# facebookresearch/videoseal

Hardware: AMD Instinct MI355X
Metric: frames/sec embed+extract 256-bit @768x768 (higher is better)
Workload: dtype f32 (2 x f16 operand split, 3 products on v_mfma_f32_32x32x16_f16, fp32 accumulate); 1 GPU; videoseal_1.0 256-bit, 32 frames 768x768 per GPU, image mode (embedder on every frame, full-res JND), embed + detect; card=videoseal_1.0, weights=random-init (seeded), no checkpoint offline, batch_per_gpu=32, mode=image

## Files before the change

### videoseal_amd/csrc/net_ops.hip

```cpp
#include <algorithm>
#include <cstdlib>
#include <cstring>

#include "conv_common.h"

namespace {

__global__ __launch_bounds__(256) void layernorm_act_kernel(const float* __restrict__ x, int64_t rows, int C, int64_t ld,
                                                            const float* __restrict__ w, const float* __restrict__ b,
                                                            float eps, int act, float* __restrict__ out, int64_t out_ld) {
  const int lane = threadIdx.x & 63;
  const int64_t row = (int64_t)blockIdx.x * 4 + (threadIdx.x >> 6);
  if (row >= rows) return;
  const float* xr = x + row * ld;
  float s = 0.f;
  for (int c = lane; c < C; c += 64) s += xr[c];
  const float mean = wave_sum(s) / (float)C;
  float v = 0.f;
  for (int c = lane; c < C; c += 64) {
    const float dlt = xr[c] - mean;
    v += dlt * dlt;
  }
  const float var = wave_sum(v) / (float)C;
  const float den = sqrtf(var + eps);
  float* orow = out + row * out_ld;
  for (int c = lane; c < (int)out_ld; c += 64) {
    float y = 0.f;
    if (c < C) y = vs_apply_act(w[c] * ((xr[c] - mean) / den) + b[c], act);
    orow[c] = y;
  }
}

template <int LPP, int VMAX>
__global__ __launch_bounds__(256) void layernorm_act_lanes_kernel(const float* __restrict__ x, int64_t rows, int C, int64_t ld,
                                                                  const float* __restrict__ w, const float* __restrict__ b, float eps, int act,
                                                                  float* __restrict__ out, int64_t out_ld, int pH, int pW) {
  constexpr int RPB = 256 / LPP;
  const int q = threadIdx.x & (LPP - 1);
  const int64_t row = (int64_t)blockIdx.x * RPB + (threadIdx.x / LPP);
  bool live = row < rows;
  const int C4 = (C + 3) >> 2, O4 = (int)(out_ld >> 2);
  const float* xr = x + (live ? row : rows - 1) * ld;
  f32x4 v[VMAX];
  float s = 0.f;
#pragma unroll
  for (int k = 0; k < VMAX; ++k) {
    const int c4 = q + k * LPP;
    v[k] = f32x4{0.f, 0.f, 0.f, 0.f};
    if (c4 < C4) {
      v[k] = *reinterpret_cast<const f32x4*>(xr + 4 * c4);
#pragma unroll
      for (int e = 0; e < 4; ++e)
        if (4 * c4 + e < C) s += v[k][e];
    }
  }
#pragma unroll
  for (int o = LPP / 2; o > 0; o >>= 1) s += __shfl_xor(s, o, 64);
  const float mean = s / (float)C;
  float qv = 0.f;
#pragma unroll
  for (int k = 0; k < VMAX; ++k) {
    const int c4 = q + k * LPP;
    if (c4 < C4) {
#pragma unroll
      for (int e = 0; e < 4; ++e)
        if (4 * c4 + e < C) { const float dlt = v[k][e] - mean; qv += dlt * dlt; }
    }
  }
#pragma unroll
  for (int o = LPP / 2; o > 0; o >>= 1) qv += __shfl_xor(qv, o, 64);
  const float den = sqrtf(qv / (float)C + eps);
  float* orow = out + row * out_ld;
  if (pW > 0 && live) {
    const int px = (int)(row % pW);
    const int64_t t = row / pW;
    const int py = (int)(t % pH);
    const int64_t fb = t / pH;
    const int oh = pH >> 1, ow = pW >> 1;
    live = (py >> 1) < oh && (px >> 1) < ow;
    orow = out + ((fb * oh + (py >> 1)) * ow + (px >> 1)) * (4 * (int64_t)C) + ((py & 1) * 2 + (px & 1)) * C;
  }
  if (!live) return;
#pragma unroll
  for (int k = 0; k < VMAX; ++k) {
    const int c4 = q + k * LPP;
    if (c4 < O4) {
      f32x4 o = {0.f, 0.f, 0.f, 0.f};
// ... 505 lines not shown

template <int CG>
__global__ __launch_bounds__(256) void upconv_gather_ln_kernel(const float* __restrict__ z, int64_t zld, int H, int W, int Co,
                                                               int tpp_log2, const float* __restrict__ lnw,
                                                               const float* __restrict__ lnb, float eps, int act,
                                                               float* __restrict__ out, int64_t old, int64_t npix, int nblk) {
  const int per = (nblk + 7) >> 3;
  const int64_t vb = (int64_t)(blockIdx.x & 7) * per + (blockIdx.x >> 3);
  const int64_t gid = vb * 256 + threadIdx.x;
  const int64_t pq = gid >> tpp_log2;
  const int g = (int)(gid & ((1 << tpp_log2) - 1));
  const bool live = pq < npix && vb < nblk;
  const int64_t p = live ? pq : 0;
  constexpr int NVP = CG / 4;
  f32x4 lwv[NVP], lbv[NVP];
#pragma unroll
  for (int j = 0; j < NVP; ++j) {
    lwv[j] = *reinterpret_cast<const f32x4*>(lnw + g * CG + 4 * j);
    lbv[j] = *reinterpret_cast<const f32x4*>(lnb + g * CG + 4 * j);
  }
  const int W2 = 2 * W, H2 = 2 * H;
  const int X = (int)(p % W2);
  const int64_t t0 = p / W2;
  const int Y = (int)(t0 % H2);
  const int64_t b = t0 / H2;
  int ys[3][2], xs[3][2];
  float wy[3][2], wx[3][2];
#pragma unroll
  for (int k = 0; k < 3; ++k) {
    int yr = Y + k - 1, xr = X + k - 1;
    yr = yr < 0 ? -yr : (yr >= H2 ? 2 * H2 - 2 - yr : yr);
    xr = xr < 0 ? -xr : (xr >= W2 ? 2 * W2 - 2 - xr : xr);
    const float sy = fmaxf((yr + 0.5f) * 0.5f - 0.5f, 0.f), sx = fmaxf((xr + 0.5f) * 0.5f - 0.5f, 0.f);
    const int y0 = (int)sy, x0 = (int)sx;
    ys[k][0] = y0; ys[k][1] = y0 + (y0 < H - 1);
    xs[k][0] = x0; xs[k][1] = x0 + (x0 < W - 1);
    wy[k][1] = sy - y0; wy[k][0] = 1.f - wy[k][1];
    wx[k][1] = sx - x0; wx[k][0] = 1.f - wx[k][1];
  }
  constexpr int NV = CG / 4;
  f32x4 acc[NV];
#pragma unroll
  for (int j = 0; j < NV; ++j) acc[j] = f32x4{0.f, 0.f, 0.f, 0.f};
  const float* zb = z + b * H * W * zld + g * CG;
#pragma unroll
  for (int ky = 0; ky < 3; ++ky)
#pragma unroll
    for (int a = 0; a < 2; ++a) {
      const float* zr = zb + (int64_t)ys[ky][a] * W * zld + ky * 3 * Co;
#pragma unroll
      for (int kx = 0; kx < 3; ++kx)
#pragma unroll
        for (int c = 0; c < 2; ++c) {
          const float w = wy[ky][a] * wx[kx][c];
          const float* q = zr + (int64_t)xs[kx][c] * zld + kx * Co;
#pragma unroll
          for (int j = 0; j < NV; ++j) acc[j] += w * *reinterpret_cast<const f32x4*>(q + 4 * j);
        }
    }
  float s = 0.f;
#pragma unroll
  for (int j = 0; j < NV; ++j) s += (acc[j][0] + acc[j][1]) + (acc[j][2] + acc[j][3]);
  for (int o = 1; o < (1 << tpp_log2); o <<= 1) s += __shfl_xor(s, o, 64);
  const float mean = s / (float)Co;
  float v = 0.f;
#pragma unroll
  for (int j = 0; j < NV; ++j)
#pragma unroll
    for (int e = 0; e < 4; ++e) { const float dl = acc[j][e] - mean; v += dl * dl; }
  for (int o = 1; o < (1 << tpp_log2); o <<= 1) v += __shfl_xor(v, o, 64);
  const float den = sqrtf(v / (float)Co + eps);
  if (!live) return;
  float* orow = out + p * old + g * CG;
#pragma unroll
  for (int j = 0; j < NV; ++j) {
    const f32x4 wv = lwv[j], bv = lbv[j];
    f32x4 o;
#pragma unroll
    for (int e = 0; e < 4; ++e) o[e] = vs_apply_act(wv[e] * ((acc[j][e] - mean) / den) + bv[e], act);
    *reinterpret_cast<f32x4*>(orow + 4 * j) = o;
  }
}

__global__ __launch_bounds__(256) void im2col3x3_kernel(const float* __restrict__ x, int H, int W, int64_t ld, int reflect,
                                                        float* __restrict__ out, int64_t total) {
  const int G = (int)(ld >> 2);
  for (int64_t i = (int64_t)blockIdx.x * 256 + threadIdx.x; i < total; i += (int64_t)gridDim.x * 256) {
    const int cg = (int)(i % G);
    int64_t r = i / G;
    const int t = (int)(r % 9);
    r /= 9;
    const int xx = (int)(r % W);
    const int yy = (int)((r / W) % H);
    const int64_t b = r / ((int64_t)W * H);
    int sy = yy + t / 3 - 1, sx = xx + t % 3 - 1;
    bool ok = true;
    if (reflect) {
      sy = sy < 0 ? -sy : (sy >= H ? 2 * H - 2 - sy : sy);
      sx = sx < 0 ? -sx : (sx >= W ? 2 * W - 2 - sx : sx);
    } else {
      ok = sy >= 0 && sy < H && sx >= 0 && sx < W;
    }
    f32x4 v = {0.f, 0.f, 0.f, 0.f};
    if (ok) v = *reinterpret_cast<const f32x4*>(x + ((b * H + sy) * W + sx) * ld + cg * 4);
    *reinterpret_cast<f32x4*>(out + (r * 9 + t) * ld + cg * 4) = v;
  }
}

__global__ __launch_bounds__(256) void msg_pre_kernel(const float* __restrict__ P, int N, float* __restrict__ T, int64_t total) {
  for (int64_t i = (int64_t)blockIdx.x * 256 + threadIdx.x; i < total; i += (int64_t)gridDim.x * 256) {
    const int n = (int)(i % N);
    const int cls = (int)((i / N) % 9);
    const int64_t bm = i / ((int64_t)9 * N);
    const int cy = cls / 3, cx = cls % 3;
    const float* pb = P + bm * 9 * N + n;
    float v = 0.f;
    for (int ky = (cy == 0 ? 1 : 0); ky <= (cy == 2 ? 1 : 2); ++ky)
      for (int kx = (cx == 0 ? 1 : 0); kx <= (cx == 2 ? 1 : 2); ++kx) v += pb[(ky * 3 + kx) * N];
    T[i] = v;
  }
}

__global__ __launch_bounds__(256) void cat2_scale_kernel(const float* __restrict__ x, int C1, int64_t ld1, const float* __restrict__ skip,
                                                         int C2, int64_t ld2, float s, int64_t rows, float* __restrict__ out,
                                                         int64_t old) {
  const int g1 = x ? C1 >> 2 : 0, G = g1 + (C2 >> 2);
  const int64_t total = rows * G;
  for (int64_t i = (int64_t)blockIdx.x * 256 + threadIdx.x; i < total; i += (int64_t)gridDim.x * 256) {
    const int cg = (int)(i % G);
    const int64_t r = i / G;
    f32x4 v;
    int c;
    if (cg < g1) { c = cg * 4; v = *reinterpret_cast<const f32x4*>(x + r * ld1 + c); }
    else { const int c2 = (cg - g1) * 4; c = C1 + c2; v = *reinterpret_cast<const f32x4*>(skip + r * ld2 + c2) * s; }
    *reinterpret_cast<f32x4*>(out + r * old + c) = v;
  }
}

__global__ __launch_bounds__(256) void msg_latent_kernel(const float* __restrict__ table, const int32_t* __restrict__ msgs,
                                                         int nbits, int hidden, float* __restrict__ lat) {
  __shared__ int rowsel[1024];
  const int b = blockIdx.y;
  for (int k = threadIdx.x; k < nbits; k += 256) rowsel[k] = 2 * k + (msgs[(int64_t)b * nbits + k] != 0);
  __syncthreads();
  const int c = blockIdx.x * 256 + threadIdx.x;
  if (c >= hidden) return;
  float s = 0.f;
  int k = 0;
  for (; k + 16 <= nbits; k += 16) {
    float v[16];
#pragma unroll
    for (int j = 0; j < 16; ++j) v[j] = table[(int64_t)rowsel[k + j] * hidden + c];
#pragma unroll
    for (int j = 0; j < 16; ++j) s += v[j];
  }
  for (; k < nbits; ++k) s += table[(int64_t)rowsel[k] * hidden + c];
  lat[(int64_t)b * hidden + c] = s;
}
__global__ __launch_bounds__(256) void broadcast_channels4_kernel(const float* __restrict__ lat, int Bm, int hidden4,
                                                                  float* __restrict__ dst, int HW, int64_t ld, int coff,
                                                                  int64_t total4) {
  for (int64_t i = (int64_t)blockIdx.x * 256 + threadIdx.x; i < total4; i += (int64_t)gridDim.x * 256) {
    const int c4 = (int)(i % hidden4);
    const int64_t p = i / hidden4;
    const int b = (int)(p / HW);
    *reinterpret_cast<f32x4*>(dst + p * ld + coff + 4 * c4) = *reinterpret_cast<const f32x4*>(lat + ((int64_t)(Bm == 1 ? 0 : b) * hidden4 + c4) * 4);
// ... 512 lines not shown
        }
    }
#pragma unroll
    for (int j = 0; j < CPT; ++j) {
      const int c = cb + threadIdx.x + 1024 * j;
      if (c < C) {
        const float gx = sqrtf(s[j]);
        scale[(int64_t)b * sld + c] = gx;
        local += gx;
      }
    }
  }
  red[threadIdx.x] = local;
  __syncthreads();
  for (int o = 512; o > 0; o >>= 1) {
    if ((int)threadIdx.x < o) red[threadIdx.x] += red[threadIdx.x + o];
    __syncthreads();
  }
  const float mean = red[0] / (float)C;
  for (int c = threadIdx.x; c < (int)sld; c += 1024) {
    float v = 0.f;
    if (c < C) v = 1.0f + gamma[c] * (scale[(int64_t)b * sld + c] / (mean + 1e-6f));
    scale[(int64_t)b * sld + c] = v;
  }
}

extern "C" int vs_grn_scale_from_straddle_partials(const float* partial, int B, int HW, int C, const float* gamma, float* scale,
                                                   int64_t scale_ld, void* stream) {
  VS_REQUIRE(partial && gamma && scale && B > 0 && HW >= 32 && C > 0 && scale_ld >= C);
  hipLaunchKernelGGL(grn_finish_straddle_kernel, dim3((unsigned)B), dim3(1024), 0, (hipStream_t)stream, partial, HW, C, gamma, scale, scale_ld);
  return vs_launch_status();
}

extern "C" int vs_upcat2x(const float* x, int C1, int64_t ld1, const float* skip, int C2, int64_t ld2, float skip_scale,
                          int B, int H, int W, float* out, int64_t out_ld, void* stream) {
  VS_REQUIRE(x && skip && out && C1 > 0 && C2 > 0 && C1 % 4 == 0 && C2 % 4 == 0 && ld1 % 4 == 0 && ld2 % 4 == 0);
  VS_REQUIRE(out_ld % 4 == 0 && out_ld >= C1 + C2 && B > 0 && H > 0 && W > 0);
  const int64_t total = (int64_t)B * 2 * H * 2 * W * (out_ld / 4);
  hipLaunchKernelGGL(upcat2x_kernel, dim3(grid_for(total, 256, 1 << 20)), dim3(256), 0, (hipStream_t)stream, x, C1, ld1, skip,
                     C2, ld2, skip_scale, B, H, W, out, out_ld, total);
  return vs_launch_status();
}

extern "C" int vs_cat2_scale(const float* x, int C1, int64_t ld1, const float* skip, int C2, int64_t ld2, float skip_scale,
                             int64_t rows, float* out, int64_t out_ld, void* stream) {
  VS_REQUIRE(skip && out && rows > 0 && C1 >= 0 && C2 > 0 && C1 % 4 == 0 && C2 % 4 == 0 && ld2 % 4 == 0 && out_ld % 4 == 0 &&
             out_ld >= C1 + C2 && (!x || (ld1 % 4 == 0 && ld1 >= C1)));
  const int64_t total = rows * ((x ? C1 : 0) + C2) / 4;
  hipLaunchKernelGGL(cat2_scale_kernel, dim3((unsigned)std::min<int64_t>(cdiv64(total, 256), 1 << 16)), dim3(256), 0, (hipStream_t)stream,
                     x, C1, ld1, skip, C2, ld2, skip_scale, rows, out, out_ld);
  return vs_launch_status();
}

extern "C" int vs_im2col3x3(const float* x, int B, int H, int W, int64_t ld, int pad_mode, float* out, void* stream) {
  VS_REQUIRE(x && out && B > 0 && H > 1 && W > 1 && ld > 0 && ld % 4 == 0);
  const int64_t total = (int64_t)B * H * W * 9 * (ld / 4);
  hipLaunchKernelGGL(im2col3x3_kernel, dim3((unsigned)std::min<int64_t>(cdiv64(total, 256), 1 << 16)), dim3(256), 0, (hipStream_t)stream, x, H,
                     W, ld, pad_mode == VS_PAD_REFLECT ? 1 : 0, out, total);
  return vs_launch_status();
}

extern "C" int vs_msg_pre(const float* P, int Bm, int N, float* table, void* stream) {
  VS_REQUIRE(P && table && Bm > 0 && N > 0);
  const int64_t total = (int64_t)Bm * 9 * N;
  hipLaunchKernelGGL(msg_pre_kernel, dim3((unsigned)std::min<int64_t>(cdiv64(total, 256), 1 << 16)), dim3(256), 0, (hipStream_t)stream, P, N, table,
                     total);
  return vs_launch_status();
}

extern "C" int vs_upconv_supported(int Co) {
  if (Co < 16 || Co % 16) return 0;
  const int cg = Co >= 64 ? 16 : Co / 4;
  const int tpp = Co / cg;
  return (cg == 4 || cg == 8 || cg == 16) && tpp <= 64 && (tpp & (tpp - 1)) == 0;
}

extern "C" int vs_upconv_gather_ln(const float* z, int64_t z_ld, int B, int H, int W, int Co, const float* lnw, const float* lnb,
                                   float eps, int act, float* out, int64_t out_ld, void* stream) {
  VS_REQUIRE(z && lnw && lnb && out && B > 0 && H > 0 && W > 0 && vs_upconv_supported(Co) && z_ld >= 9 * (int64_t)Co && z_ld % 4 == 0 &&
             out_ld >= Co && out_ld % 4 == 0);
  const int cg = Co >= 64 ? 16 : Co / 4;
  int tl = 0;
  while ((cg << tl) < Co) ++tl;
  const int64_t npix = (int64_t)B * 4 * H * W;
  const int64_t nblk64 = cdiv64(npix << tl, 256);
  VS_REQUIRE(nblk64 < (1 << 30));
  const int nblk = (int)nblk64;
  const int grid = ((nblk + 7) / 8) * 8;
  hipStream_t st = (hipStream_t)stream;
#define VS_UPG(CG_) hipLaunchKernelGGL(upconv_gather_ln_kernel<CG_>, dim3(grid), dim3(256), 0, st, z, z_ld, H, W, Co, tl, lnw, lnb, eps, act, out, out_ld, npix, nblk)
  if (cg == 4) VS_UPG(4);
  else if (cg == 8) VS_UPG(8);
  else VS_UPG(16);
#undef VS_UPG
  return vs_launch_status();
}

extern "C" int vs_msg_latent(const float* table, const int32_t* msgs, int Bm, int nbits, int hidden, float* lat, void* stream) {
  VS_REQUIRE(table && msgs && lat && Bm > 0 && nbits > 0 && nbits <= 1024 && hidden > 0);
  hipLaunchKernelGGL(msg_latent_kernel, dim3((unsigned)((hidden + 255) / 256), (unsigned)Bm), dim3(256), 0, (hipStream_t)stream,
                     table, msgs, nbits, hidden, lat);
  return vs_launch_status();
}

extern "C" int vs_broadcast_channels(const float* lat, int Bm, int hidden, float* dst, int B, int HW, int64_t ld, int coff,
                                     void* stream) {
  VS_REQUIRE(lat && dst && (Bm == 1 || Bm == B) && hidden > 0 && B > 0 && HW > 0 && coff >= 0 && coff + hidden <= ld);
  const int64_t total = (int64_t)B * HW * hidden;
  if ((hidden & 3) == 0 && (ld & 3) == 0 && (coff & 3) == 0 && (((uintptr_t)lat | (uintptr_t)dst) & 15) == 0) {
    hipLaunchKernelGGL(broadcast_channels4_kernel, dim3(grid_for(total / 4, 256, 1 << 20)), dim3(256), 0, (hipStream_t)stream, lat, Bm,
                       hidden / 4, dst, HW, ld, coff, total / 4);
    return vs_launch_status();
  }
  hipLaunchKernelGGL(broadcast_channels_kernel, dim3(grid_for(total, 256, 1 << 20)), dim3(256), 0, (hipStream_t)stream, lat, Bm,
                     hidden, dst, HW, ld, coff, total);
  return vs_launch_status();
}

extern "C" int vs_outc_tanh(const float* x, int64_t rows_per_frame, int B, int C, int64_t ld, const float* w, const float* bias,
                            int Cout, int use_tanh, float* out, void* stream) {
  VS_REQUIRE(x && w && bias && out && rows_per_frame > 0 && B > 0 && C > 0 && ld % 4 == 0 && ld >= C && Cout > 0 && Cout <= 4);
  const int64_t rows = rows_per_frame * B;
  hipLaunchKernelGGL(outc_tanh_kernel, dim3((unsigned)cdiv64(rows, 256)), dim3(256), 0, (hipStream_t)stream, x, rows_per_frame,
                     rows, C, ld, w, bias, Cout, use_tanh, out);
  return vs_launch_status();
}

extern "C" int vs_pool_linear(const float* x, int B, int HW, int C, int64_t ld, const float* w, const float* bias, int N,
                              float* out, void* stream) {
  VS_REQUIRE(x && w && bias && out && B > 0 && HW > 0 && C > 0 && ld >= C && N > 0);
  const size_t smem = (size_t)C * sizeof(float);
  if (smem > 64 * 1024) return VS_ERR_UNSUPPORTED;
  hipLaunchKernelGGL(pool_linear_kernel, dim3((unsigned)B, 16), dim3(256), smem, (hipStream_t)stream, x, HW, C, ld, w, bias, N, out);
  return vs_launch_status();
}

extern "C" int64_t vs_bn_partial_doubles(int64_t rows, int64_t ld) { return ld >= 4 ? cdiv64(rows, bn_chunk_rows(ld)) * 2 * ld : 0; }

extern "C" int vs_bn_batch_stats(const float* x, int64_t rows, int C, int64_t ld, const float* gamma, const float* beta, float eps,
                                 float momentum, float* running_mean, float* running_var, double* partial, float* scale, float* shift,
                                 void* stream) {
  VS_REQUIRE(x && gamma && beta && partial && scale && shift && rows > 0 && C > 0 && ld >= C && (ld & 3) == 0);
  VS_REQUIRE((((uintptr_t)x) & 15) == 0);
  const int nchunk = (int)cdiv64(rows, bn_chunk_rows(ld));
  launch_bn_partial(x, rows, ld, partial, (hipStream_t)stream);
  hipLaunchKernelGGL(bn_finish_kernel, dim3((unsigned)C), dim3(64), 0, (hipStream_t)stream, partial, nchunk, rows, C, ld,
                     gamma, beta, eps, momentum, running_mean, running_var, scale, shift, (const double*)nullptr);
  return vs_launch_status();
}

extern "C" int vs_bn_partial_sums(const float* x, int64_t rows, int C, int64_t ld, double* partial, double* sums, void* stream) {
  VS_REQUIRE(x && partial && sums && rows > 0 && C > 0 && ld >= C && (ld & 3) == 0);
  VS_REQUIRE((((uintptr_t)x) & 15) == 0);
  const int nchunk = (int)cdiv64(rows, bn_chunk_rows(ld));
  launch_bn_partial(x, rows, ld, partial, (hipStream_t)stream);
  hipLaunchKernelGGL(bn_reduce_kernel, dim3((unsigned)ld), dim3(64), 0, (hipStream_t)stream, partial, nchunk, rows, ld, sums);
  return vs_launch_status();
}

extern "C" int vs_bn_finish_sums(const double* sums, int C, int64_t ld, const float* gamma, const float* beta, float eps, float momentum,
                                 float* running_mean, float* running_var, float* scale, float* shift, void* stream) {
  VS_REQUIRE(sums && gamma && beta && scale && shift && C > 0 && ld >= C);
  hipLaunchKernelGGL(bn_finish_kernel, dim3((unsigned)C), dim3(64), 0, (hipStream_t)stream, sums, 1, (int64_t)0, C, ld,
                     gamma, beta, eps, momentum, running_mean, running_var, scale, shift, sums + 2 * ld);
  return vs_launch_status();
}

extern "C" int vs_scale_shift_act(const float* x, int64_t rows, int C, int64_t ld, const float* scale, const float* shift, int act,
                                  const float* add, int64_t add_ld, float* out, int64_t out_ld, void* stream) {
  VS_REQUIRE(x && scale && shift && out && rows > 0 && C > 0 && (C & 3) == 0 && ld >= C && out_ld >= C && (ld & 3) == 0 && (out_ld & 3) == 0);
  VS_REQUIRE(!add || (add_ld >= C && (add_ld & 3) == 0));
  hipLaunchKernelGGL(scale_shift_act_kernel, dim3(grid_for(rows * (C >> 2), 256, 1 << 16)), dim3(256), 0, (hipStream_t)stream, x, rows, C,
                     ld, scale, shift, act, add, add_ld, out, out_ld);
  return vs_launch_status();
}

// ... 16 lines not shown
```

### videoseal_amd/csrc/upconv_fused.hip

```cpp
#include <algorithm>
#include <cstdlib>

#include "conv_common.h"

namespace {

using namespace vsconv;

constexpr int UT = 8;
constexpr int UH = UT + 2;
constexpr int UROWS = 128;

template <int NB, int CG, int NP>
__global__ __launch_bounds__(256, (NB <= 5 ? 2 : 1)) void upconv_fused_kernel(const float* __restrict__ x, int C1, int64_t ld1, const float* __restrict__ skip,
                                                           int C2, int64_t ld2, float sscale, const unsigned short* __restrict__ wsplit,
                                                           int H, int W, int Co, const float* __restrict__ lnw,
                                                           const float* __restrict__ lnb, float eps, int act, float* __restrict__ out,
                                                           int64_t old, int tiles_x, int tiles_y, int nblk, int abl, float a_mul, float acc_mul) {
  using AR = Arith<NP>;
  constexpr int BN = NB * 32;
  constexpr int A_BYTES = NP * UROWS * ROWB;
  extern __shared__ __attribute__((aligned(16))) unsigned char smem_u[];
  unsigned char* const As = smem_u;
  unsigned char* const Bs = smem_u + A_BYTES;
  float* const Z = reinterpret_cast<float*>(smem_u);
  const int N = 9 * Co, K = C1 + C2, ZS = N + 4;
  const int tid = threadIdx.x, lane = tid & 63, wave = tid >> 6;
  const int r = lane & 31, g = lane >> 5;
  const int per = (nblk + 7) >> 3;
  const int vb = (blockIdx.x & 7) * per + (blockIdx.x >> 3);
  if (vb >= nblk) return;
  const int tx = vb % tiles_x;
  const int t1 = vb / tiles_x;
  const int ty = t1 % tiles_y;
  const int b = t1 / tiles_y;
  const int y0 = ty * UT - 1, x0 = tx * UT - 1;

  int64_t a_pix[2];
  int a_lds[2];
#pragma unroll
  for (int i = 0; i < 2; ++i) {
    const int s = tid + i * 256;
    const int row = s >> 2;
    const int hy = row < UH * UH ? row / UH : 0, hx = row < UH * UH ? row % UH : 0;
    const int py = min(max(y0 + hy, 0), H - 1), px = min(max(x0 + hx, 0), W - 1);
    a_pix[i] = ((int64_t)b * H + py) * W + px;
    a_lds[i] = row * ROWB + (s & 3) * 8;
  }
  const int k4 = (tid & 3) * 4;
  constexpr int BSLOT = BN * 2;
  constexpr int NBL = (BSLOT + 255) / 256;

  f32x16 acc[NB];
#pragma unroll
  for (int j = 0; j < NB; ++j)
#pragma unroll
    for (int e = 0; e < 16; ++e) acc[j][e] = 0.f;

  constexpr int KG = NB <= 5 ? 4 : 8;
  u32x4 rb[NBL][NP];
  auto fetch_b = [&](const int kc) __attribute__((always_inline)) {
#pragma unroll
    for (int i = 0; i < NBL; ++i) {
      const int s = tid + i * 256;
      const int row = s >> 1, sub = s & 1;
#pragma unroll
      for (int p = 0; p < NP; ++p) {
        rb[i][p] = u32x4{0u, 0u, 0u, 0u};
        if (s < BSLOT && row < N) rb[i][p] = *reinterpret_cast<const u32x4*>(wsplit + ((int64_t)p * N + row) * K + kc + sub * 8);
      }
    }
  };
  fetch_b(0);
  for (int kg = 0; kg < ((abl & 1) ? 0 : K); kg += KG * BK) {
    f32x4 ra[KG][2];
#pragma unroll
    for (int c = 0; c < KG; ++c) {
      const int kc = kg + c * BK < K ? kg + c * BK : K - BK;
      const bool from_x = kc < C1;
      const float mul = from_x ? 1.0f : sscale;
#pragma unroll
      for (int i = 0; i < 2; ++i) {
        const float* src = from_x ? x + a_pix[i] * ld1 + kc + k4 : skip + a_pix[i] * ld2 + (kc - C1) + k4;
        ra[c][i] = *reinterpret_cast<const f32x4*>(src) * mul;
      }
    }
#pragma unroll
    for (int c = 0; c < KG; ++c) {
      const int kc = kg + c * BK;
      if (kc < K) {
        if (kc) __syncthreads();
#pragma unroll
        for (int i = 0; i < 2; ++i) {
          u32x2 pl[NP];
          split4n<NP>(ra[c][i], a_mul, pl);
#pragma unroll
          for (int p = 0; p < NP; ++p) *reinterpret_cast<u32x2*>(As + p * UROWS * ROWB + a_lds[i]) = pl[p];
        }
#pragma unroll
        for (int i = 0; i < NBL; ++i) {
          const int s = tid + i * 256;
          if (s < BSLOT) {
#pragma unroll
            for (int p = 0; p < NP; ++p) *reinterpret_cast<u32x4*>(Bs + p * BN * ROWB + (s >> 1) * ROWB + (s & 1) * 16) = rb[i][p];
          }
        }
        __syncthreads();
        if (kc + BK < K) fetch_b(kc + BK);
        bf16x8 af[NP], bf[NB][NP];
#pragma unroll
        for (int p = 0; p < NP; ++p) af[p] = *reinterpret_cast<const bf16x8*>(As + p * UROWS * ROWB + (wave * 32 + r) * ROWB + g * 16);
#pragma unroll
        for (int j = 0; j < NB; ++j)
#pragma unroll
          for (int p = 0; p < NP; ++p) bf[j][p] = *reinterpret_cast<const bf16x8*>(Bs + p * BN * ROWB + (j * 32 + r) * ROWB + g * 16);
#pragma unroll
        for (int q = 0; q < AR::NPROD; ++q) {
#pragma unroll
          for (int j = 0; j < NB; ++j) acc[j] = AR::mfma(af[AR::PA[q]], bf[j][AR::PB[q]], acc[j]);
        }
      }
    }
  }
  __syncthreads();
#pragma unroll
  for (int j = 0; j < NB; ++j) {
    const int n = j * 32 + r;
#pragma unroll
    for (int e = 0; e < 16; ++e) {
      const int m = wave * 32 + (e & 3) + 8 * (e >> 2) + 4 * g;
      if (m < UH * UH && n < N) Z[m * ZS + n] = NP == 2 ? acc[j][e] * acc_mul : acc[j][e];
    }
  }
  __syncthreads();

  constexpr int NV = CG / 4;
  const int q4 = tid & 3;
  f32x4 lwv[NV], lbv[NV];
#pragma unroll
  for (int j = 0; j < NV; ++j) {
    lwv[j] = *reinterpret_cast<const f32x4*>(lnw + q4 * CG + 4 * j);
    lbv[j] = *reinterpret_cast<const f32x4*>(lnb + q4 * CG + 4 * j);
  }
  const int H2 = 2 * H, W2 = 2 * W;
  const float invC = 1.0f / (float)Co;
  for (int it = tid >> 2; it < ((abl & 2) ? 0 : 4 * UT * UT); it += 64) {
    const int oy = it / (2 * UT), ox = it % (2 * UT);
    const int Y = (y0 + 1) * 2 + oy, X = (x0 + 1) * 2 + ox;
    const bool live = Y < H2 && X < W2;
    const int Yc = min(Y, H2 - 1), Xc = min(X, W2 - 1);
    int ys[3][2], xs[3][2];
    float wy[3][2], wx[3][2];
#pragma unroll
    for (int k = 0; k < 3; ++k) {
      int yr = Yc + k - 1, xr = Xc + k - 1;
      yr = yr < 0 ? -yr : (yr >= H2 ? 2 * H2 - 2 - yr : yr);
      xr = xr < 0 ? -xr : (xr >= W2 ? 2 * W2 - 2 - xr : xr);
      const float sy = fmaxf((yr + 0.5f) * 0.5f - 0.5f, 0.f), sx = fmaxf((xr + 0.5f) * 0.5f - 0.5f, 0.f);
      const int yl = (int)sy, xl = (int)sx;
      ys[k][0] = yl - y0; ys[k][1] = yl + (yl < H - 1) - y0;
      xs[k][0] = xl - x0; xs[k][1] = xl + (xl < W - 1) - x0;
      wy[k][1] = sy - yl; wy[k][0] = 1.f - wy[k][1];
      wx[k][1] = sx - xl; wx[k][0] = 1.f - wx[k][1];
    }
    f32x4 v[NV];
#pragma unroll
    for (int j = 0; j < NV; ++j) v[j] = f32x4{0.f, 0.f, 0.f, 0.f};
    const float* zb = Z + q4 * CG;
#pragma unroll
    for (int ky = 0; ky < 3; ++ky)
#pragma unroll
      for (int a = 0; a < 2; ++a) {
        const float* zr = zb + ys[ky][a] * UH * ZS + ky * 3 * Co;
#pragma unroll
        for (int kx = 0; kx < 3; ++kx)
#pragma unroll
          for (int c = 0; c < 2; ++c) {
            const float w = wy[ky][a] * wx[kx][c];
            const float* qz = zr + xs[kx][c] * ZS + kx * Co;
#pragma unroll
            for (int j = 0; j < NV; ++j) v[j] += w * *reinterpret_cast<const f32x4*>(qz + 4 * j);
          }
      }
    float s = 0.f;
#pragma unroll
    for (int j = 0; j < NV; ++j) s += (v[j][0] + v[j][1]) + (v[j][2] + v[j][3]);
    s += __shfl_xor(s, 1, 64);
    s += __shfl_xor(s, 2, 64);
    const float mean = s * invC;
    float var = 0.f;
#pragma unroll
    for (int j = 0; j < NV; ++j)
#pragma unroll
      for (int e = 0; e < 4; ++e) { const float dl = v[j][e] - mean; var += dl * dl; }
    var += __shfl_xor(var, 1, 64);
    var += __shfl_xor(var, 2, 64);
    const float den = sqrtf(var * invC + eps);
    if (!live) continue;
    float* orow = out + (((int64_t)b * H2 + Y) * W2 + X) * old + q4 * CG;
#pragma unroll
    for (int j = 0; j < NV; ++j) {
      const f32x4 wv = lwv[j], bv = lbv[j];
      f32x4 o;
#pragma unroll
      for (int e = 0; e < 4; ++e) o[e] = vs_apply_act(wv[e] * ((v[j][e] - mean) / den) + bv[e], act);
      *reinterpret_cast<f32x4*>(orow + 4 * j) = o;
    }
  }
}

template <int NB, int CG>
int launch_fused(const float* x, int C1, int64_t ld1, const float* skip, int C2, int64_t ld2, float s, const void* wsplit, int B, int H, int W,
                 int Co, const float* lnw, const float* lnb, float eps, int act, float* out, int64_t old, int arith, float a_mul, float acc_mul,
                 hipStream_t st) {
  const size_t stage = 3 * (size_t)(UROWS + NB * 32) * ROWB, ztile = (size_t)UH * UH * (9 * Co + 4) * sizeof(float);
  const size_t smem = std::max(stage, ztile);
  if (smem > 160 * 1024) return VS_ERR_UNSUPPORTED;
  auto kern = arith == 2 ? upconv_fused_kernel<NB, CG, 2> : upconv_fused_kernel<NB, CG, 3>;
  static bool attr[2] = {false, false};
  if (smem > 64 * 1024 && !attr[arith == 2]) {
    (void)hipFuncSetAttribute((const void*)kern, hipFuncAttributeMaxDynamicSharedMemorySize, 160 * 1024);
    attr[arith == 2] = true;
  }
  const int tiles_x = (W + UT - 1) / UT, tiles_y = (H + UT - 1) / UT;
  const int64_t nblk = (int64_t)B * tiles_x * tiles_y;
  if (nblk >= (1 << 30)) return VS_ERR_UNSUPPORTED;
  static const int abl = [] { const char* e = getenv("VS_UPCONV_ABL"); return e ? atoi(e) : 0; }();
  hipLaunchKernelGGL(kern, dim3((unsigned)((nblk + 7) / 8 * 8)), dim3(256), smem, st, x, C1, ld1, skip, C2, ld2, s,
                     static_cast<const unsigned short*>(wsplit), H, W, Co, lnw, lnb, eps, act, out, old, tiles_x, tiles_y, (int)nblk, abl, a_mul, acc_mul);
  return vs_launch_status();
}

}

extern "C" int vs_upconv_fused_supported(int C1, int C2, int Co) {
  return (Co == 16 || Co == 32) && C1 > 0 && C2 > 0 && C1 % 16 == 0 && C2 % 16 == 0 && C1 + C2 <= 256;
}
extern "C" int vs_upconv_fused_preferred(int C1, int C2, int Co) { return vs_upconv_fused_supported(C1, C2, Co) && Co == 16; }

extern "C" int vs_upconv_fused(const float* x, int C1, int64_t ld1, const float* skip, int C2, int64_t ld2, float skip_scale,
                               const void* wt_split, int B, int H, int W, int Co, const float* lnw, const float* lnb, float eps, int act,
                               float* out, int64_t out_ld, int arith, float a_mul, float acc_mul, void* stream) {
  VS_REQUIRE((arith == 0 || arith == 3) || (arith == 2 && a_mul > 0.f && acc_mul > 0.f));
  VS_REQUIRE(x && skip && wt_split && lnw && lnb && out && B > 0 && H > 0 && W > 0 && vs_upconv_fused_supported(C1, C2, Co));
  VS_REQUIRE(ld1 % 4 == 0 && ld2 % 4 == 0 && ld1 >= C1 && ld2 >= C2 && out_ld % 4 == 0 && out_ld >= Co && ((uintptr_t)wt_split & 15) == 0);
  hipStream_t st = (hipStream_t)stream;
  if (Co == 16) return launch_fused<5, 4>(x, C1, ld1, skip, C2, ld2, skip_scale, wt_split, B, H, W, Co, lnw, lnb, eps, act, out, out_ld, arith, a_mul, acc_mul, st);
  return launch_fused<9, 8>(x, C1, ld1, skip, C2, ld2, skip_scale, wt_split, B, H, W, Co, lnw, lnb, eps, act, out, out_ld, arith, a_mul, acc_mul, st);
}
```

### videoseal_amd/csrc/vs_common.h

```cpp
#pragma once
#include <hip/hip_runtime.h>
#include <stdint.h>
#include <stdlib.h>
#include <string.h>

#include "videoseal_hip.h"

typedef float f32x4 __attribute__((ext_vector_type(4)));
typedef float f32x16 __attribute__((ext_vector_type(16)));

#define VS_REQUIRE(cond)                  \
  do {                                    \
    if (!(cond)) return VS_ERR_BAD_ARG;   \
  } while (0)

static inline int vs_launch_status() { return hipGetLastError() == hipSuccess ? VS_OK : VS_ERR_LAUNCH; }

static inline int64_t cdiv64(int64_t a, int64_t b) { return (a + b - 1) / b; }

#define VS_DEFAULT_ARITH 2
static inline int vs_default_arith() {
  static const int a = [] {
    const char* e = getenv("VIDEOSEAL_CONV");
    if (e && !strcmp(e, "f16x2")) return 2;
    if (e && !strcmp(e, "bf16x3")) return 3;
    return VS_DEFAULT_ARITH;
  }();
  return a;
}

enum { VS_DBG_RESIZE_FORM = 0 , VS_DBG_RESIZE_STRIP = 1 , VS_DBG_TAIL_STRIP = 2 , VS_DBG_JPEG_FORM = 3 , VS_DBG_CROP_RESIZE_FORM = 4 , VS_DBG_TO_PLANES_FORM = 5 , VS_DBG_DWCONV_ROWS = 6 , VS_DBG_LN_FORM = 7 , VS_DBG_SPLITK_EPI = 8 , VS_DBG_COUNT = 9 };
int vs_debug_get(int key);

static inline int vs_max_lds_bytes() {
  static const int n = [] {
    int dev = 0, v = 0;
    if (hipGetDevice(&dev) != hipSuccess || hipDeviceGetAttribute(&v, hipDeviceAttributeMaxSharedMemoryPerBlock, dev) != hipSuccess || v <= 0) v = 64 * 1024;
    return v;
  }();
  return n;
}

static inline int vs_num_cus() {
  static const int n = [] {
    int dev = 0, v = 0;
    if (hipGetDevice(&dev) != hipSuccess || hipDeviceGetAttribute(&v, hipDeviceAttributeMultiprocessorCount, dev) != hipSuccess || v <= 0) v = 256;
    return v;
  }();
  return n;
}

__device__ __forceinline__ float vs_erfc_sqrt2(float a) {
  const float u = fminf(a, 5.65685424949238f);
  float q = 5.128553084e-07f;
  q = __builtin_fmaf(q, u, -9.560153558e-06f);
  q = __builtin_fmaf(q, u, 7.497344632e-05f);
  q = __builtin_fmaf(q, u, -2.843466646e-04f);
  q = __builtin_fmaf(q, u, 1.498938855e-05f);
  q = __builtin_fmaf(q, u, 6.931120995e-03f);
  q = __builtin_fmaf(q, u, -5.243476480e-02f);
  q = __builtin_fmaf(q, u, -4.592214525e-01f);
  q = __builtin_fmaf(q, u, -1.151104212e+00f);
  return __builtin_amdgcn_exp2f(q * u);
}
__device__ __forceinline__ float vs_gelu(float v) {
  const float a = fabsf(v);
  const float e = vs_erfc_sqrt2(a);
  return fmaxf(v, 0.f) - (0.5f * a) * e;
}
typedef float vs_f32x2 __attribute__((ext_vector_type(2)));
__device__ __forceinline__ vs_f32x2 vs_gelu2(const vs_f32x2 v) {
#pragma clang fp contract(off)
  const vs_f32x2 a = {fabsf(v[0]), fabsf(v[1])};
  const vs_f32x2 u = {fminf(a[0], 5.65685424949238f), fminf(a[1], 5.65685424949238f)};
  vs_f32x2 q = {5.128553084e-07f, 5.128553084e-07f};
  q = __builtin_elementwise_fma(q, u, vs_f32x2{-9.560153558e-06f, -9.560153558e-06f});
  q = __builtin_elementwise_fma(q, u, vs_f32x2{7.497344632e-05f, 7.497344632e-05f});
  q = __builtin_elementwise_fma(q, u, vs_f32x2{-2.843466646e-04f, -2.843466646e-04f});
  q = __builtin_elementwise_fma(q, u, vs_f32x2{1.498938855e-05f, 1.498938855e-05f});
  q = __builtin_elementwise_fma(q, u, vs_f32x2{6.931120995e-03f, 6.931120995e-03f});
  q = __builtin_elementwise_fma(q, u, vs_f32x2{-5.243476480e-02f, -5.243476480e-02f});
  q = __builtin_elementwise_fma(q, u, vs_f32x2{-4.592214525e-01f, -4.592214525e-01f});
  q = __builtin_elementwise_fma(q, u, vs_f32x2{-1.151104212e+00f, -1.151104212e+00f});
  const vs_f32x2 t = q * u;
  const vs_f32x2 e = {__builtin_amdgcn_exp2f(t[0]), __builtin_amdgcn_exp2f(t[1])};
  const vs_f32x2 m = {fmaxf(v[0], 0.f), fmaxf(v[1], 0.f)};
  return __builtin_elementwise_fma(a * -0.5f, e, m);
}
__device__ __forceinline__ float vs_gelu_grad(float v) {
  const float e = vs_erfc_sqrt2(fabsf(v));
  const float Phi = v >= 0.f ? 1.f - 0.5f * e : 0.5f * e;
  return Phi + v * (0.3989422804014327f * __expf(-0.5f * v * v));
}

__device__ __forceinline__ float vs_relu(float v) { return v <= 0.f ? 0.f : v; }

__device__ __forceinline__ float vs_apply_act(float v, int act) {
  switch (act) {
    case VS_ACT_RELU: return vs_relu(v);
    case VS_ACT_GELU: return vs_gelu(v);
    case VS_ACT_TANH: return tanhf(v);
    case VS_ACT_SILU: return v / (1.0f + __expf(-v));
    default: return v;
  }
}

__device__ __forceinline__ float wave_sum(float v) {
#pragma unroll
  for (int o = 32; o > 0; o >>= 1) v += __shfl_xor(v, o, 64);
  return v;
}
```

Before: 4239 frames/s.

## Gather upconv outputs per 2x2 output block to share bilinear taps

Adds a shared helper that computes the four upsampled outputs belonging to one low-res cell together. It reuses the overlapping bilinear-resize and 3x3 taps across the 2x2 quad, with software-prefetched loads. The helper is used both in the standalone gather+LayerNorm kernel and in the fused upconv epilogue, and becomes the default path. The old per-pixel path stays reachable through a debug switch. The goal is fewer redundant loads and FMAs, in exchange for more registers per thread (2x2xNV accumulators) and possible occupancy loss.

```diff
diff --git a/videoseal_amd/csrc/net_ops.hip b/videoseal_amd/csrc/net_ops.hip
--- a/videoseal_amd/csrc/net_ops.hip
+++ b/videoseal_amd/csrc/net_ops.hip
@@ -3,6 +3,7 @@
 #include <cstring>
 
 #include "conv_common.h"
+#include "upconv_gather.h"
 
 namespace {
 
@@ -674,6 +675,76 @@
   }
 }
 
+template <int CG>
+__global__ __launch_bounds__(256) void upconv_gather_ln_blk_kernel(const float* __restrict__ z, int64_t zld, int H, int W, int Co,
+                                                                   int tpp_log2, const float* __restrict__ lnw,
+                                                                   const float* __restrict__ lnb, float eps, int act,
+                                                                   float* __restrict__ out, int64_t old, int64_t ncell, int nblk) {
+  const int per = (nblk + 7) >> 3;
+  const int64_t vb = (int64_t)(blockIdx.x & 7) * per + (blockIdx.x >> 3);
+  const int64_t gid = vb * 256 + threadIdx.x;
+  const int64_t cq = gid >> tpp_log2;
+  const int g = (int)(gid & ((1 << tpp_log2) - 1));
+  const bool live = cq < ncell && vb < nblk;
+  const int64_t cell = live ? cq : 0;
+  constexpr int NV = CG / 4;
+  f32x4 lwv[NV], lbv[NV];
+#pragma unroll
+  for (int j = 0; j < NV; ++j) {
+    lwv[j] = *reinterpret_cast<const f32x4*>(lnw + g * CG + 4 * j);
+    lbv[j] = *reinterpret_cast<const f32x4*>(lnb + g * CG + 4 * j);
+  }
+  const int x = (int)(cell % W);
+  const int64_t t0 = cell / W;
+  const int y = (int)(t0 % H);
+  const int64_t b = t0 / H;
+  UpAxis ay, ax;
+  upconv_axis(y, H, ay);
+  upconv_axis(x, W, ax);
+  f32x4 acc[2][2][NV];
+#pragma unroll
+  for (int p = 0; p < 2; ++p)
+#pragma unroll
+    for (int q = 0; q < 2; ++q)
+#pragma unroll
+      for (int j = 0; j < NV; ++j) acc[p][q][j] = f32x4{0.f, 0.f, 0.f, 0.f};
+  upconv_gather_2x2<NV, int64_t>(z + b * H * W * zld + g * CG, (int64_t)W * zld, zld, Co, ay, ax, acc);
+  float mean[2][2], den[2][2];
+#pragma unroll
+  for (int p = 0; p < 2; ++p)
+#pragma unroll
+    for (int q = 0; q < 2; ++q) {
+      float s = 0.f;
+#pragma unroll
+      for (int j = 0; j < NV; ++j) s += (acc[p][q][j][0] + acc[p][q][j][1]) + (acc[p][q][j][2] + acc[p][q][j][3]);
+      for (int o = 1; o < (1 << tpp_log2); o <<= 1) s += __shfl_xor(s, o, 64);
+      mean[p][q] = s / (float)Co;
+      float v = 0.f;
+#pragma unroll
+      for (int j = 0; j < NV; ++j)
+#pragma unroll
+        for (int e = 0; e < 4; ++e) { const float dl = acc[p][q][j][e] - mean[p][q]; v += dl * dl; }
+      for (int o = 1; o < (1 << tpp_log2); o <<= 1) v += __shfl_xor(v, o, 64);
+      den[p][q] = sqrtf(v / (float)Co + eps);
+    }
+  if (!live) return;
+  const int64_t W2 = 2 * (int64_t)W;
+#pragma unroll
+  for (int p = 0; p < 2; ++p)
+#pragma unroll
+    for (int q = 0; q < 2; ++q) {
+      float* orow = out + (((b * 2 * H + 2 * y + p) * W2) + 2 * x + q) * old + g * CG;
+#pragma unroll
+      for (int j = 0; j < NV; ++j) {
+        const f32x4 wv = lwv[j], bv = lbv[j];
+        f32x4 o;
+#pragma unroll
+        for (int e = 0; e < 4; ++e) o[e] = vs_apply_act(wv[e] * ((acc[p][q][j][e] - mean[p][q]) / den[p][q]) + bv[e], act);
+        *reinterpret_cast<f32x4*>(orow + 4 * j) = o;
+      }
+    }
+}
+
 __global__ __launch_bounds__(256) void im2col3x3_kernel(const float* __restrict__ x, int H, int W, int64_t ld, int reflect,
                                                         float* __restrict__ out, int64_t total) {
   const int G = (int)(ld >> 2);
@@ -1352,16 +1423,23 @@
   const int cg = Co >= 64 ? 16 : Co / 4;
   int tl = 0;
   while ((cg << tl) < Co) ++tl;
-  const int64_t npix = (int64_t)B * 4 * H * W;
-  const int64_t nblk64 = cdiv64(npix << tl, 256);
+  const bool blocked = vs_debug_get(VS_DBG_UPCONV_FORM) != 1;
+  const int64_t nitem = (int64_t)B * H * W * (blocked ? 1 : 4);
+  const int64_t nblk64 = cdiv64(nitem << tl, 256);
   VS_REQUIRE(nblk64 < (1 << 30));
   const int nblk = (int)nblk64;
   const int grid = ((nblk + 7) / 8) * 8;
   hipStream_t st = (hipStream_t)stream;
-#define VS_UPG(CG_) hipLaunchKernelGGL(upconv_gather_ln_kernel<CG_>, dim3(grid), dim3(256), 0, st, z, z_ld, H, W, Co, tl, lnw, lnb, eps, act, out, out_ld, npix, nblk)
-  if (cg == 4) VS_UPG(4);
-  else if (cg == 8) VS_UPG(8);
-  else VS_UPG(16);
+#define VS_UPG(KERN_, CG_) hipLaunchKernelGGL(KERN_<CG_>, dim3(grid), dim3(256), 0, st, z, z_ld, H, W, Co, tl, lnw, lnb, eps, act, out, out_ld, nitem, nblk)
+  if (blocked) {
+    if (cg == 4) VS_UPG(upconv_gather_ln_blk_kernel, 4);
+    else if (cg == 8) VS_UPG(upconv_gather_ln_blk_kernel, 8);
+    else VS_UPG(upconv_gather_ln_blk_kernel, 16);
+  } else {
+    if (cg == 4) VS_UPG(upconv_gather_ln_kernel, 4);
+    else if (cg == 8) VS_UPG(upconv_gather_ln_kernel, 8);
+    else VS_UPG(upconv_gather_ln_kernel, 16);
+  }
 #undef VS_UPG
   return vs_launch_status();
 }
diff --git a/videoseal_amd/csrc/upconv_fused.hip b/videoseal_amd/csrc/upconv_fused.hip
--- a/videoseal_amd/csrc/upconv_fused.hip
+++ b/videoseal_amd/csrc/upconv_fused.hip
@@ -2,6 +2,7 @@
 #include <cstdlib>
 
 #include "conv_common.h"
+#include "upconv_gather.h"
 
 namespace {
 
@@ -144,6 +145,60 @@
   }
   const int H2 = 2 * H, W2 = 2 * W;
   const float invC = 1.0f / (float)Co;
+  if (!(abl & 4)) {
+    if (abl & 2) return;
+    const int cy = tid >> 5, cx = (tid >> 2) & (UT - 1);
+    const int yc = y0 + 1 + cy, xc = x0 + 1 + cx;
+    const bool live = yc < H && xc < W;
+    UpAxis ay, ax;
+    upconv_axis(min(yc, H - 1), H, ay);
+    upconv_axis(min(xc, W - 1), W, ax);
+#pragma unroll
+    for (int p = 0; p < 2; ++p)
+#pragma unroll
+      for (int k = 0; k < 3; ++k)
+#pragma unroll
+        for (int a = 0; a < 2; ++a) { ay.s[p][k][a] -= y0; ax.s[p][k][a] -= x0; }
+    f32x4 v[2][2][NV];
+#pragma unroll
+    for (int p = 0; p < 2; ++p)
+#pragma unroll
+      for (int q = 0; q < 2; ++q)
+#pragma unroll
+        for (int j = 0; j < NV; ++j) v[p][q][j] = f32x4{0.f, 0.f, 0.f, 0.f};
+    upconv_gather_2x2<NV, int>(Z + q4 * CG, UH * ZS, ZS, Co, ay, ax, v);
+#pragma unroll
+    for (int p = 0; p < 2; ++p)
+#pragma unroll
+      for (int q = 0; q < 2; ++q) {
+        float s = 0.f;
+#pragma unroll
+        for (int j = 0; j < NV; ++j) s += (v[p][q][j][0] + v[p][q][j][1]) + (v[p][q][j][2] + v[p][q][j][3]);
+        s += __shfl_xor(s, 1, 64);
+        s += __shfl_xor(s, 2, 64);
+        const float mean = s * invC;
+        float var = 0.f;
+#pragma unroll
+        for (int j = 0; j < NV; ++j)
+#pragma unroll
+          for (int e = 0; e < 4; ++e) { const float dl = v[p][q][j][e] - mean; var += dl * dl; }
+        var += __shfl_xor(var, 1, 64);
+        var += __shfl_xor(var, 2, 64);
+        const float den = sqrtf(var * invC + eps);
+        if (live) {
+          float* orow = out + (((int64_t)b * H2 + 2 * yc + p) * W2 + 2 * xc + q) * old + q4 * CG;
+#pragma unroll
+          for (int j = 0; j < NV; ++j) {
+            const f32x4 wv = lwv[j], bv = lbv[j];
+            f32x4 o;
+#pragma unroll
+            for (int e = 0; e < 4; ++e) o[e] = vs_apply_act(wv[e] * ((v[p][q][j][e] - mean) / den) + bv[e], act);
+            *reinterpret_cast<f32x4*>(orow + 4 * j) = o;
+          }
+        }
+      }
+    return;
+  }
   for (int it = tid >> 2; it < ((abl & 2) ? 0 : 4 * UT * UT); it += 64) {
     const int oy = it / (2 * UT), ox = it % (2 * UT);
     const int Y = (y0 + 1) * 2 + oy, X = (x0 + 1) * 2 + ox;
@@ -226,8 +281,9 @@
   const int64_t nblk = (int64_t)B * tiles_x * tiles_y;
   if (nblk >= (1 << 30)) return VS_ERR_UNSUPPORTED;
   static const int abl = [] { const char* e = getenv("VS_UPCONV_ABL"); return e ? atoi(e) : 0; }();
+  const int form = vs_debug_get(VS_DBG_UPCONV_FORM) == 1 ? 4 : 0;
   hipLaunchKernelGGL(kern, dim3((unsigned)((nblk + 7) / 8 * 8)), dim3(256), smem, st, x, C1, ld1, skip, C2, ld2, s,
-                     static_cast<const unsigned short*>(wsplit), H, W, Co, lnw, lnb, eps, act, out, old, tiles_x, tiles_y, (int)nblk, abl, a_mul, acc_mul);
+                     static_cast<const unsigned short*>(wsplit), H, W, Co, lnw, lnb, eps, act, out, old, tiles_x, tiles_y, (int)nblk, abl | form, a_mul, acc_mul);
   return vs_launch_status();
 }
 
diff --git a/videoseal_amd/csrc/upconv_gather.h b/videoseal_amd/csrc/upconv_gather.h
--- /dev/null
+++ b/videoseal_amd/csrc/upconv_gather.h
@@ -0,0 +1,93 @@
+#pragma once
+#include <utility>
+
+#include "vs_common.h"
+
+struct UpAxis {
+  int s[2][3][2];
+  float w[2][3][2];
+  bool k1_b0_is_a1;
+  bool k2_a0_is_b0;
+};
+
+__device__ __forceinline__ void upconv_axis(const int cell, const int n, UpAxis& ax) {
+  const int n2 = 2 * n;
+#pragma unroll
+  for (int p = 0; p < 2; ++p)
+#pragma unroll
+    for (int k = 0; k < 3; ++k) {
+      int r = 2 * cell + p + k - 1;
+      r = r < 0 ? -r : (r >= n2 ? 2 * n2 - 2 - r : r);
+      const float sf = fmaxf((r + 0.5f) * 0.5f - 0.5f, 0.f);
+      const int i0 = (int)sf;
+      ax.s[p][k][0] = i0; ax.s[p][k][1] = i0 + (i0 < n - 1);
+      ax.w[p][k][1] = sf - i0; ax.w[p][k][0] = 1.f - ax.w[p][k][1];
+    }
+  ax.k1_b0_is_a1 = ax.s[1][1][0] == ax.s[0][1][1];
+  ax.k2_a0_is_b0 = ax.s[0][2][0] == ax.s[1][2][0];
+}
+
+__device__ __forceinline__ int upconv_item(const UpAxis& ax, const int k, const int i) {
+  return k == 0 ? ax.s[0][0][i] : k == 1 ? (i < 2 ? ax.s[0][1][i] : ax.s[1][1][1]) : (i == 0 ? ax.s[1][2][0] : ax.s[0][2][1]);
+}
+
+template <class F, int... I>
+__device__ __forceinline__ void upconv_static_for(F&& f, std::integer_sequence<int, I...>) { (f(std::integral_constant<int, I>{}), ...); }
+
+template <int NV, class Off>
+__device__ __forceinline__ void upconv_gather_2x2(const float* __restrict__ zb, const Off rs, const Off cs, const int Co, const UpAxis& ay,
+                                                  const UpAxis& ax, f32x4 (&acc)[2][2][NV]) {
+  constexpr int NSTEP = 7 * NV;
+  constexpr bool AHEAD = NV <= 2;
+  f32x4 zbuf[AHEAD ? 2 : 1][3][3];
+  auto load = [&](const int t, f32x4 (&zc)[3][3]) __attribute__((always_inline)) {
+    const int r7 = t / NV, j = t % NV;
+    const int ky = r7 < 2 ? 0 : (r7 < 5 ? 1 : 2), ri = r7 - (ky == 0 ? 0 : (ky == 1 ? 2 : 5));
+    const float* zr = zb + (Off)upconv_item(ay, ky, ri) * rs + ky * 3 * Co + 4 * j;
+#pragma unroll
+    for (int kx = 0; kx < 3; ++kx)
+#pragma unroll
+      for (int ci = 0; ci < (kx == 1 ? 3 : 2); ++ci) zc[kx][ci] = *reinterpret_cast<const f32x4*>(zr + (Off)upconv_item(ax, kx, ci) * cs + kx * Co);
+  };
+  if (AHEAD) load(0, zbuf[0]);
+  upconv_static_for([&](auto tc) __attribute__((always_inline)) {
+    constexpr int t = decltype(tc)::value;
+    constexpr int cur = AHEAD ? (t & 1) : 0;
+    if (!AHEAD) load(t, zbuf[0]);
+    else if (t + 1 < NSTEP) load(t + 1, zbuf[AHEAD ? ((t + 1) & 1) : 0]);
+    __builtin_amdgcn_sched_barrier(0);
+    constexpr int r7 = t / NV, j = t % NV;
+    constexpr int ky = r7 < 2 ? 0 : (r7 < 5 ? 1 : 2), ri = r7 - (ky == 0 ? 0 : (ky == 1 ? 2 : 5));
+    const f32x4 (&zc)[3][3] = zbuf[cur];
+    const f32x4 z_k1b0 = ax.k1_b0_is_a1 ? zc[1][1] : zc[1][0];
+    const f32x4 z_k2a0 = ax.k2_a0_is_b0 ? zc[2][0] : zc[2][1];
+    auto sweep = [&](const int p, const int a, const bool on) __attribute__((always_inline)) {
+      const float wyv = ay.w[p][ky][a];
+#pragma unroll
+      for (int kx = 0; kx < 3; ++kx)
+#pragma unroll
+        for (int c = 0; c < 2; ++c) {
+          const f32x4 z0 = c == 1 ? zc[kx][1] : (kx == 2 ? z_k2a0 : zc[kx][0]);
+          const f32x4 z1 = kx == 1 ? (c == 1 ? zc[1][2] : z_k1b0) : zc[kx][c];
+          const f32x4 t0 = acc[p][0][j] + (wyv * ax.w[0][kx][c]) * z0;
+          const f32x4 t1 = acc[p][1][j] + (wyv * ax.w[1][kx][c]) * z1;
+          acc[p][0][j] = on ? t0 : acc[p][0][j];
+          acc[p][1][j] = on ? t1 : acc[p][1][j];
+        }
+    };
+    if (ky == 0) {
+      sweep(0, ri, true);
+      sweep(1, ri, true);
+    } else if (ky == 1) {
+      if (ri == 0) { sweep(0, 0, true); sweep(1, 0, !ay.k1_b0_is_a1); }
+      if (ri == 1) { sweep(0, 1, true); sweep(1, 0, ay.k1_b0_is_a1); }
+      if (ri == 2) sweep(1, 1, true);
+    } else {
+      if (ri == 0) { sweep(1, 0, true); sweep(0, 0, ay.k2_a0_is_b0); }
+      if (ri == 1) { sweep(0, 0, !ay.k2_a0_is_b0); sweep(0, 1, true); sweep(1, 1, true); }
+    }
+#pragma unroll
+    for (int p = 0; p < 2; ++p) asm volatile("" : "+v"(acc[p][0][j]), "+v"(acc[p][1][j]));
+    __builtin_amdgcn_sched_barrier(0);
+  }, std::make_integer_sequence<int, NSTEP>{});
+}
diff --git a/videoseal_amd/csrc/vs_common.h b/videoseal_amd/csrc/vs_common.h
--- a/videoseal_amd/csrc/vs_common.h
+++ b/videoseal_amd/csrc/vs_common.h
@@ -29,7 +29,7 @@
   return a;
 }
 
-enum { VS_DBG_RESIZE_FORM = 0 , VS_DBG_RESIZE_STRIP = 1 , VS_DBG_TAIL_STRIP = 2 , VS_DBG_JPEG_FORM = 3 , VS_DBG_CROP_RESIZE_FORM = 4 , VS_DBG_TO_PLANES_FORM = 5 , VS_DBG_DWCONV_ROWS = 6 , VS_DBG_LN_FORM = 7 , VS_DBG_SPLITK_EPI = 8 , VS_DBG_COUNT = 9 };
+enum { VS_DBG_RESIZE_FORM = 0 , VS_DBG_RESIZE_STRIP = 1 , VS_DBG_TAIL_STRIP = 2 , VS_DBG_JPEG_FORM = 3 , VS_DBG_CROP_RESIZE_FORM = 4 , VS_DBG_TO_PLANES_FORM = 5 , VS_DBG_DWCONV_ROWS = 6 , VS_DBG_LN_FORM = 7 , VS_DBG_SPLITK_EPI = 8 , VS_DBG_UPCONV_FORM = 9 , VS_DBG_COUNT = 10 };
 int vs_debug_get(int key);
 
 static inline int vs_max_lds_bytes() {
```

Measured after the change: 4285 frames/s (median of 6 runs). 1.1% higher.
